# 2gunsu/monocon-pytorch

Measured on AMD Instinct MI355X. Metric: images/sec (384x1280) fwd+bwd, higher is better.
Workload: dtype f32 (f16x2); 1 GPU; train step B=32/GPU 3x384x1280 (configs[2] shape, fp32 values, mode f16x2); global_batch=32, parallelism=dp1, precision_mode=f16x2

## Files before the change

monocon-pytorch_amd/csrc/kernels_head_train.hip:

```cpp
#include <type_traits>

#include "kernels.h"
#include "train.h"

namespace mc {

__global__ void pack_conv_w_dgrad_kernel(const float *__restrict__ w, int Cout, int CinTotal, int k, int c_off, int Cs,
                                         int CsP, int CoutPad, int cls, float *__restrict__ dst) {
    const int kk = k * k;
    const size_t total = (size_t)Cout * Cs * kk;
    const int py = cls >> 1, px = cls & 1;
    for (size_t e = blockIdx.x * (size_t)blockDim.x + threadIdx.x; e < total; e += (size_t)gridDim.x * blockDim.x) {
        const int tap = e % kk;
        const int cl = (e / kk) % Cs;
        const int n = e / ((size_t)kk * Cs);
        const int r = tap / k, s = tap % k;
        int tapd;
        if (cls < 0) {
            tapd = (k - 1 - r) * k + (k - 1 - s);
        } else {
            if ((py == 0) != (r == 1) || (px == 0) != (s == 1)) continue;
            const int dr = py ? (2 - r) / 2 : 0, ds = px ? (2 - s) / 2 : 0;
            tapd = dr * (1 + px) + ds;
        }
        dst[(((size_t)tapd * (CoutPad >> 2) + (n >> 2)) * CsP + cl) * 4 + (n & 3)] =
            w[(((size_t)n * CinTotal + c_off + cl) * k + r) * k + s];
    }
}
hipError_t launch_pack_conv_w_dgrad(const float *w, int Cout, int CinTotal, int k, int c_off, int Cs, int CsP, int CoutPad,
                                    int cls, float *dst, hipStream_t st) {
    const size_t total = (size_t)Cout * Cs * k * k;
    size_t g = (total + 255) / 256;
    if (g > 4096) g = 4096;
    hipLaunchKernelGGL(pack_conv_w_dgrad_kernel, dim3((unsigned)g), dim3(256), 0, st, w, Cout, CinTotal, k, c_off, Cs, CsP,
                       CoutPad, cls, dst);
    return hipGetLastError();
}

struct HeadBwdArgs {
    const float *draw; int ld;
    const float *z, *x, *w1;
    const float *scale, *shift;
    float *d, *dw_partial, *red_partial;
    int HW, rows_per_block, blocks_per_img;
    const float *coef;
    float *csum;
    unsigned *amax;
};
constexpr int HB_PX = 64, HB_LD = 80;
constexpr int HB_WAVES = 4, HB_NT = HB_WAVES * 64, HB_MAXR = 24;

template <int RB, int NR, int MODE>
struct HeadPart {
    static constexpr int CP = NUM_HEADS * HEAD_CH;
    float w[NR], acc[NR];
    float s1, s2, zsc, zsh, cp, cq, cr;
    const float *xp, *zp;
    float *dp;
    bool rez;
    int h, sub, nsub;

    __device__ __forceinline__ void init(const HeadBwdArgs &a, int h_, int lane, size_t p0, int b, int sub_, int nsub_) {
        h = h_; sub = sub_; nsub = nsub_;
#pragma unroll
        for (int r = 0; r < NR; ++r) { w[r] = a.w1[(RB + r) * HEAD_CH + lane]; acc[r] = 0.f; }
        s1 = 0.f; s2 = 0.f;
        rez = a.z == nullptr;
        zsc = rez ? a.scale[(size_t)b * CP + h * HEAD_CH + lane] : 0.f;
        zsh = rez ? a.shift[(size_t)b * CP + h * HEAD_CH + lane] : 0.f;
        xp = a.x + p0 * CP + h * HEAD_CH + lane;
        zp = rez ? xp : a.z + p0 * CP + h * HEAD_CH + lane;
        dp = MODE == 1 ? nullptr : a.d + p0 * CP + h * HEAD_CH + lane;
        cp = cq = cr = 0.f;
        if (MODE == 2) {
            const float4 cf = reinterpret_cast<const float4 *>(a.coef)[(size_t)b * CP + h * HEAD_CH + lane];
            cp = cf.x; cq = cf.y; cr = cf.z;
        }
    }
    __device__ __forceinline__ void one(const float *gsh, int i, size_t gp, float zv, float xv) {
        const float *g = gsh + i * NR;
        float dh = 0.f;
#pragma unroll
        for (int r = 0; r < NR; ++r) {
            const float gv = g[r];
            if (MODE != 2) acc[r] = fmaf(gv, zv, acc[r]);
            dh = fmaf(gv, w[r], dh);
        }
        const float dv = zv > 0.f ? dh : 0.f;
        if (MODE == 2) {
            const float o = fmaf(cp, dv, fmaf(cq, xv, cr));
            s1 += o;
            s2 = fmaxf(s2, fabsf(o));
            dp[gp * CP] = o;
        } else {
            s1 += dv;
            s2 = fmaf(dv, xv, s2);
            if (MODE == 0) dp[gp * CP] = dv;
        }
    }
    __device__ __forceinline__ void block(const float *gsh, int px0, int n) {
        constexpr int U = NR > 8 ? 4 : 8;
        const int cnt = n > sub ? (n - sub + nsub - 1) / nsub : 0;
        int k = 0;
        for (; k + U <= cnt; k += U) {
            float zv[U], xv[U];
#pragma unroll
            for (int u = 0; u < U; ++u) {
                const size_t gp = (size_t)(px0 + sub + (k + u) * nsub);
                xv[u] = xp[gp * CP];
                if (!rez) zv[u] = zp[gp * CP];
            }
#pragma unroll
            for (int u = 0; u < U; ++u) {
                const int i = sub + (k + u) * nsub;
                one(gsh, i, (size_t)(px0 + i), rez ? fmaxf(fmaf(xv[u], zsc, zsh), 0.f) : zv[u], xv[u]);
                if (NR > 8) __builtin_amdgcn_sched_barrier(0);
            }
        }
        for (; k < cnt; ++k) {
            const int i = sub + k * nsub;
            const size_t gp = (size_t)(px0 + i);
            const float xv1 = xp[gp * CP];
            one(gsh, i, gp, rez ? fmaxf(fmaf(xv1, zsc, zsh), 0.f) : zp[gp * CP], xv1);
        }
    }
    __device__ __forceinline__ void spill(float *red, int lane) const {
        if (nsub == 1 || sub == 0) return;
        float *q = red + (size_t)(sub - 1) * (NR + 2) * 64 + lane;
        if (MODE != 2) {
#pragma unroll
            for (int r = 0; r < NR; ++r) q[r * 64] = acc[r];
        }
        q[NR * 64] = s1;
        q[(NR + 1) * 64] = s2;
    }
    __device__ __forceinline__ void finish(const HeadBwdArgs &a, const float *red, int blk, int lane) {
        if (MODE == 2 && a.amax) amax_update_wave(a.amax, s2);
        if (sub != 0) return;
        for (int k = 1; k < nsub; ++k) {
            const float *q = red + (size_t)(k - 1) * (NR + 2) * 64 + lane;
            if (MODE != 2) {
#pragma unroll
                for (int r = 0; r < NR; ++r) acc[r] += q[r * 64];
                s2 += q[(NR + 1) * 64];
            }
            s1 += q[NR * 64];
        }
        if (MODE == 2) {
            a.csum[((size_t)blk * CP + h * HEAD_CH + lane) * 2] = s1;
            return;
        }
#pragma unroll
        for (int r = 0; r < NR; ++r) a.dw_partial[((size_t)blk * NUM_OUT_ROWS + RB + r) * HEAD_CH + lane] = acc[r];
        float *rp = a.red_partial + ((size_t)blk * CP + h * HEAD_CH + lane) * 2;
        rp[0] = s1;
        rp[1] = s2;
    }
};

template <int RB, int NR, int MODE>
__device__ __forceinline__ void head_bwd_one(const HeadBwdArgs &a, float *gsh, float *red, int h, int wv, int lane, size_t p0, int np,
                                             int blk, int b) {
    HeadPart<RB, NR, MODE> P;
    P.init(a, h, lane, p0, b, wv, HB_WAVES);
    constexpr int NE = HB_PX * NR, NL = (NE + HB_NT - 1) / HB_NT;
    const int tid = threadIdx.x;
    const float *gsrc = a.draw + p0 * a.ld + RB;
    float pre[NL];
    auto fetch = [&](int px0) {
#pragma unroll
        for (int k = 0; k < NL; ++k) {
            const int e = tid + k * HB_NT, px = e / NR, r = e % NR;
            pre[k] = (e < NE && px0 + px < np) ? gsrc[(size_t)(px0 + px) * a.ld + r] : 0.f;
        }
    };
    fetch(0);
    for (int px0 = 0; px0 < np; px0 += HB_PX) {
        __syncthreads();
#pragma unroll
        for (int k = 0; k < NL; ++k) {
            const int e = tid + k * HB_NT;
            if (e < NE) gsh[e] = pre[k];
        }
        __syncthreads();
        if (px0 + HB_PX < np) fetch(px0 + HB_PX);
        P.block(gsh, px0, min(HB_PX, np - px0));
    }
    P.spill(red, lane);
    __syncthreads();
    P.finish(a, red, blk, lane);
}
template <int MODE, bool WIDE>
__global__ __launch_bounds__(HB_NT) void head_bwd_kernel(const HeadBwdArgs a) {
    __shared__ float gsh[HB_PX * (WIDE ? HB_MAXR : 3)];
    __shared__ float red[(HB_WAVES - 1) * ((WIDE ? HB_MAXR : 3) + 2) * 64];
    const int lane = threadIdx.x & 63;
    const int wv = __builtin_amdgcn_readfirstlane(threadIdx.x >> 6);
    const int blk = blockIdx.x;
    const int b = blk / a.blocks_per_img, rb = blk % a.blocks_per_img;
    const int r0 = rb * a.rows_per_block;
    const int np = min(a.HW, r0 + a.rows_per_block) - r0;
    const size_t p0 = (size_t)b * a.HW + r0;
    if (WIDE) {
        switch (blockIdx.y) {
            case 0: head_bwd_one<41, 24, MODE>(a, gsh, red, 8, wv, lane, p0, np, blk, b); break;
            case 1: head_bwd_one<7, 18, MODE>(a, gsh, red, 3, wv, lane, p0, np, blk, b); break;
            default: head_bwd_one<25, 9, MODE>(a, gsh, red, 4, wv, lane, p0, np, blk, b); break;
        }
    } else {
        switch (blockIdx.y) {
            case 0: head_bwd_one<0, 3, MODE>(a, gsh, red, 0, wv, lane, p0, np, blk, b); break;
            case 1: head_bwd_one<3, 2, MODE>(a, gsh, red, 1, wv, lane, p0, np, blk, b); break;
            case 2: head_bwd_one<5, 2, MODE>(a, gsh, red, 2, wv, lane, p0, np, blk, b); break;
            case 3: head_bwd_one<34, 2, MODE>(a, gsh, red, 5, wv, lane, p0, np, blk, b); break;
            case 4: head_bwd_one<36, 3, MODE>(a, gsh, red, 6, wv, lane, p0, np, blk, b); break;
            default: head_bwd_one<39, 2, MODE>(a, gsh, red, 7, wv, lane, p0, np, blk, b); break;
        }
    }
}
template <int MODE>
static void head_bwd_launch(const HeadBwdArgs &a, int blocks, hipStream_t st) {
    hipLaunchKernelGGL((head_bwd_kernel<MODE, true>), dim3(blocks, 3), dim3(HB_NT), 0, st, a);
    hipLaunchKernelGGL((head_bwd_kernel<MODE, false>), dim3(blocks, 6), dim3(HB_NT), 0, st, a);
}
static hipError_t head_bwd_args(HeadBwdArgs &a, const float *draw, int ld, const float *z, const float *x, const float *w1, int B,
                                int HW, int blocks, const float *scale, const float *shift) {
    const int *rbeg = head_row_begin();
    static const int RB[NUM_HEADS + 1] = {0, 3, 5, 7, 25, 34, 36, 39, 41, 65};
    for (int i = 0; i <= NUM_HEADS; ++i)
        if (rbeg[i] != RB[i]) return hipErrorInvalidValue;
    if (blocks % B || ld != HB_LD) return hipErrorInvalidValue;
    if (!z && (!scale || !shift)) return hipErrorInvalidValue;
    a = HeadBwdArgs{};
    a.draw = draw; a.ld = ld; a.z = z; a.x = x; a.w1 = w1;
    a.scale = scale; a.shift = shift;
    a.HW = HW; a.blocks_per_img = blocks / B; a.rows_per_block = (HW + a.blocks_per_img - 1) / a.blocks_per_img;
    return hipSuccess;
}
hipError_t launch_head_bwd(const float *draw, int ld, const float *z, const float *x, const float *w1, int B, int HW,
                           int blocks, float *d, float *dw_partial, float *red_partial, hipStream_t st, const float *scale,
                           const float *shift) {
    HeadBwdArgs a;
    hipError_t e = head_bwd_args(a, draw, ld, z, x, w1, B, HW, blocks, scale, shift);
    if (e != hipSuccess) return e;
    a.d = d; a.dw_partial = dw_partial; a.red_partial = red_partial;
    if (d) head_bwd_launch<0>(a, blocks, st);
    else head_bwd_launch<1>(a, blocks, st);
    return hipGetLastError();
}
hipError_t launch_head_dx(const float *draw, int ld, const float *x, const float *w1, const float *coef, int B, int HW, int blocks,
                          float *dx, float *csum, float *csum_out, unsigned *amax, hipStream_t st, const float *scale,
                          const float *shift) {
    if (!coef || !dx || !csum || !csum_out) return hipErrorInvalidValue;
    HeadBwdArgs a;
    hipError_t e = head_bwd_args(a, draw, ld, nullptr, x, w1, B, HW, blocks, scale, shift);
    if (e != hipSuccess) return e;
    a.d = dx; a.coef = coef; a.csum = csum; a.amax = amax;
    head_bwd_launch<2>(a, blocks, st);
    return launch_colsum_final(csum, blocks, NUM_HEADS * HEAD_CH, csum_out, st);
}


struct DpredPackArgs {
    const float *dpred[10];
    int ld, B, HW;
    float *out;
    int row_pred[NUM_OUT_ROWS], row_ch[NUM_OUT_ROWS], pred_c[10];
};
struct DpredUserArgs : DpredPackArgs {
    const float *grad[10];
    const float *pred[10];
    int row_epi[NUM_OUT_ROWS];
};
__device__ __forceinline__ float pred_act_grad(int epi, float y) {
    if (epi == 1) return (y > 1e-4f && y < 1.f - 1e-4f) ? y * (1.f - y) : 0.f;
    if (epi == 2) {
        const float sig = 1.f / (y + 1.f) - 1e-12f;
        return -sig * (1.f - sig) / ((sig + 1e-12f) * (sig + 1e-12f));
    }
    return 1.f;
}
template <bool USER>
__global__ __launch_bounds__(256) void dpred_pack_kernel(const std::conditional_t<USER, DpredUserArgs, DpredPackArgs> a) {
    __shared__ float t[64][NUM_OUT_ROWS + 2];
    __shared__ const float *rowp[NUM_OUT_ROWS];
    __shared__ const float *rowg[USER ? NUM_OUT_ROWS : 1], *rowy[USER ? NUM_OUT_ROWS : 1];
    __shared__ int rowe[USER ? NUM_OUT_ROWS : 1];
    const int tiles = (a.HW + 63) / 64;
    const int b = blockIdx.x / tiles, hw0 = (blockIdx.x % tiles) * 64;
    if (threadIdx.x < NUM_OUT_ROWS) {
        const int r = threadIdx.x, p = a.row_pred[r];
        rowp[r] = a.dpred[p] + ((size_t)b * a.pred_c[p] + a.row_ch[r]) * a.HW + hw0;
        if constexpr (USER) {
            const size_t o = ((size_t)b * a.pred_c[p] + a.row_ch[r]) * a.HW + hw0;
            rowg[r] = a.grad[p] ? a.grad[p] + o : nullptr;
            rowy[r] = a.pred[p] + o;
            rowe[r] = a.row_epi[r];
        }
    }
    __syncthreads();
    for (int e = threadIdx.x; e < 64 * NUM_OUT_ROWS; e += 256) {
        const int r = e / 64, px = e % 64;
        if constexpr (USER) {
            float v = 0.f;
            if (hw0 + px < a.HW) {
                v = rowp[r][px];
                if (rowg[r]) v += pred_act_grad(rowe[r], rowy[r][px]) * rowg[r][px];
            }
            t[px][r] = v;
        } else {
            t[px][r] = (hw0 + px < a.HW) ? rowp[r][px] : 0.f;
        }
    }
    __syncthreads();
    for (int e = threadIdx.x; e < 64 * a.ld; e += 256) {
        const int px = e / a.ld, r = e % a.ld;
        if (hw0 + px < a.HW) a.out[((size_t)b * a.HW + hw0 + px) * a.ld + r] = r < NUM_OUT_ROWS ? t[px][r] : 0.f;
    }
}
static void dpred_pack_args(DpredPackArgs &a, const float *const dpred[10], int ld, int B, int HW, float *out) {
    a.ld = ld; a.B = B; a.HW = HW; a.out = out;
    const HeadRow *rows = head_rows();
    for (int i = 0; i < 10; ++i) { a.dpred[i] = dpred[i]; a.pred_c[i] = PRED_CH[i]; }
    for (int r = 0; r < NUM_OUT_ROWS; ++r) { a.row_pred[r] = rows[r].pred; a.row_ch[r] = rows[r].ch; }
}
hipError_t launch_dpred_pack(const float *const dpred[10], int ld, int B, int HW, float *out, hipStream_t st) {
    DpredPackArgs a;
    dpred_pack_args(a, dpred, ld, B, HW, out);
    hipLaunchKernelGGL(dpred_pack_kernel<false>, dim3(B * ((HW + 63) / 64)), dim3(256), 0, st, a);
    return hipGetLastError();
}
hipError_t launch_dpred_pack_user(const float *const dpred[10], const float *const pred[10], const float *const grad[10], int ld,
                                  int B, int HW, float *out, hipStream_t st) {
    DpredUserArgs a;
    dpred_pack_args(a, dpred, ld, B, HW, out);
    const HeadRow *rows = head_rows();
    for (int i = 0; i < 10; ++i) {
        if (!pred[i]) return hipErrorInvalidValue;
        a.pred[i] = pred[i]; a.grad[i] = grad[i];
    }
    for (int r = 0; r < NUM_OUT_ROWS; ++r) a.row_epi[r] = rows[r].epi;
    hipLaunchKernelGGL(dpred_pack_kernel<true>, dim3(B * ((HW + 63) / 64)), dim3(256), 0, st, a);
    return hipGetLastError();
}

__device__ __forceinline__ float wave_sum(float v) {
#pragma unroll
    for (int o = 32; o > 0; o >>= 1) v += __shfl_xor(v, o);
    return v;
}

__device__ __forceinline__ void group_reduce2(double &s1, double &s2, double (*sh)[64][2], int grp, int c) {
    __syncthreads();
    sh[grp][c][0] = s1; sh[grp][c][1] = s2;
    __syncthreads();
    s1 = 0; s2 = 0;
#pragma unroll
    for (int g = 0; g < 16; ++g) { s1 += sh[g][c][0]; s2 += sh[g][c][1]; }
}

__global__ __launch_bounds__(1024) void inst_stats_kernel(const float *__restrict__ stats, int chunks, int stat_ld,
                                                          double *__restrict__ out) {
    const int b = blockIdx.x, c = threadIdx.x & 63, ch = blockIdx.y * 64 + c, part = threadIdx.x >> 6;
    const float2 *q = reinterpret_cast<const float2 *>(stats) + (size_t)b * chunks * stat_ld + ch;
    double s1 = 0.0, s2 = 0.0;
    int k = part;
    for (; k + 48 < chunks; k += 64) {
        const float2 v0 = q[(size_t)k * stat_ld], v1 = q[(size_t)(k + 16) * stat_ld], v2 = q[(size_t)(k + 32) * stat_ld],
                     v3 = q[(size_t)(k + 48) * stat_ld];
        s1 += (double)v0.x; s2 += (double)v0.y;
        s1 += (double)v1.x; s2 += (double)v1.y;
        s1 += (double)v2.x; s2 += (double)v2.y;
        s1 += (double)v3.x; s2 += (double)v3.y;
    }
    for (; k < chunks; k += 16) {
        const float2 v = q[(size_t)k * stat_ld];
        s1 += (double)v.x; s2 += (double)v.y;
    }
    __shared__ double red[2][16][64];
    red[0][part][c] = s1;
    red[1][part][c] = s2;
    __syncthreads();
    if (part < 2) {
        double t = 0.0;
#pragma unroll
        for (int g = 0; g < 16; ++g) t += red[part][g][c];
        out[((size_t)b * stat_ld + ch) * 2 + part] = t;
    }
}

__global__ __launch_bounds__(1024) void attn_train_fwd_kernel(const AttnTrainArgs a) {
    __shared__ double shred[16][64][2];
    const int h = blockIdx.x, c = threadIdx.x & 63, grp = threadIdx.x >> 6;
    const int CP = NUM_HEADS * HEAD_CH, ch = h * HEAD_CH + c;
    const double HW = (double)a.HW, n = HW * a.B;
    __shared__ float att[64][NUM_AFFINE];
    __shared__ float svl[64][HEAD_CH], awl[NUM_AFFINE][HEAD_CH];
    const float shift0 = a.rm[h][c];
    double S1 = 0, S2 = 0;
    double pre1[8], pre2[8];
    float aw[NUM_AFFINE], wk_[NUM_AFFINE], bk_[NUM_AFFINE];
#pragma unroll
    for (int k = 0; k < NUM_AFFINE; ++k) {
        aw[k] = a.att_w[h][k * HEAD_CH + c]; wk_[k] = a.weight_[h][k * HEAD_CH + c]; bk_[k] = a.bias_[h][k * HEAD_CH + c];
    }
    const int ck = c < NUM_AFFINE ? c : 0;
    const float att_g_c = a.att_g[h][ck], att_b_c = a.att_b[h][ck], att_rm_c = a.att_rm[h][ck], att_rv_c = a.att_rv[h][ck];
    const float rv_c = a.rv[h][c];
    for (int b = 0; b < a.B; ++b) {
        double s1 = 0, s2 = 0;
        if (a.stats64) {
            if ((b & 7) == 0) {
#pragma unroll
                for (int u = 0; u < 8; ++u) {
                    const int bb = b + u < a.B ? b + u : a.B - 1;
                    const double2 v = *reinterpret_cast<const double2 *>(a.stats64 + ((size_t)bb * a.stat_ld + ch) * 2);
                    pre1[u] = v.x; pre2[u] = v.y;
                }
// ... 501 lines not shown
```

monocon-pytorch_amd/csrc/mc_train_plan.hip:

```cpp
#include <atomic>
#include <deque>
#include <functional>

#include "mc_internal.h"

using namespace mc;

namespace {

using Fn = std::function<int(mc_handle *, hipStream_t)>;

struct PlanSwitches {
    long long lazy_z;
    long long lazy_min;
    long long lazy_feat;
    long long zbits;
    long long grad_pool;
    long long grad_pool_cool;
    long long head_dx_fuse;
    long long dgrad_s2_thin;
    long long stem_fuse;
    long long bm_epilogue;
    long long wres_bwd;
    long long dual_stream;
    int side_sync_lo = 0, side_sync_hi = 0;
    bool plan_debug = false;
};
const struct { const char *name; long long PlanSwitches::*field; long long def; } SWITCH_TABLE[] = {
    {"MONOCON_HIP_LAZY_Z", &PlanSwitches::lazy_z, 3},
    {"MONOCON_HIP_LAZY_MIN", &PlanSwitches::lazy_min, 900000},
    {"MONOCON_HIP_LAZY_FEAT", &PlanSwitches::lazy_feat, 0},
    {"MONOCON_HIP_ZBITS", &PlanSwitches::zbits, 1},
    {"MONOCON_HIP_GRAD_POOL", &PlanSwitches::grad_pool, 1},
    {"MONOCON_HIP_GRAD_POOL_COOL", &PlanSwitches::grad_pool_cool, 2},
    {"MONOCON_HIP_HEAD_DX_FUSE", &PlanSwitches::head_dx_fuse, 1},
    {"MONOCON_HIP_DGRAD_S2_THIN", &PlanSwitches::dgrad_s2_thin, 1},
    {"MONOCON_HIP_STEM_FUSE", &PlanSwitches::stem_fuse, 1},
    {"MONOCON_HIP_BM_EPILOGUE", &PlanSwitches::bm_epilogue, 1},
    {"MONOCON_HIP_WRES_BWD", &PlanSwitches::wres_bwd, 0},
    {"MONOCON_HIP_DUAL_STREAM", &PlanSwitches::dual_stream, 1},
};
PlanSwitches read_switches() {
    PlanSwitches sw{};
    std::string changed;
    for (const auto &d : SWITCH_TABLE) {
        const char *e = std::getenv(d.name);
        sw.*d.field = e ? std::atoll(e) : d.def;
        if (sw.*d.field != d.def) changed += std::string(" ") + d.name + "=" + std::to_string(sw.*d.field);
    }
    if (const char *e = std::getenv("MONOCON_HIP_SIDE_SYNC")) {
        if (std::sscanf(e, "%d:%d", &sw.side_sync_lo, &sw.side_sync_hi) != 2) sw.side_sync_lo = sw.side_sync_hi = 0;
        if (sw.side_sync_lo < sw.side_sync_hi) changed += std::string(" MONOCON_HIP_SIDE_SYNC=") + e;
    }
    sw.plan_debug = std::getenv("MONOCON_HIP_PLAN_DEBUG") != nullptr;
    if (sw.plan_debug && !changed.empty()) fprintf(stderr, "[plan] switches off their defaults:%s\n", changed.c_str());
    return sw;
}

struct PoolBwdArgs {
    const float *x, *dout, *la, *lb;
    float *dx, *stats;
    int B, H, W, C, acc;
};

struct LastWriter {
    enum Kind { NONE, DGRAD_CONV, POOL_BWD, DECONV_BWD } kind = NONE;
    union {
        ConvArgs *conv;
        PoolBwdArgs *pool;
        float **deconv_stats;
    };
    LastWriter() : conv(nullptr) {}
    LastWriter(ConvArgs *c) : kind(c ? DGRAD_CONV : NONE), conv(c) {}
    LastWriter(PoolBwdArgs *p) : kind(p ? POOL_BWD : NONE), pool(p) {}
    LastWriter(float **s) : kind(s ? DECONV_BWD : NONE), deconv_stats(s) {}
};

struct TNode {
    Tensor t;
    float *g = nullptr;
    bool ginit = false, needs_grad = true;
    LastWriter last;
    const float *la = nullptr, *lb = nullptr;
    bool lrelu = true;
};

struct PackJob {
    const float *w;
    int Cout, CinTotal, k, c_off, Cs, CsP, CoutPad;
    int cls;
    float *dst;
    void *dst16;
    unsigned *amax;
};

enum RecKind { REC_STEM, REC_CONV, REC_POOL, REC_DECONV, REC_HEAD };
struct Rec {
    RecKind kind;
    ConvLayer *L = nullptr;
    DeconvLayer *D = nullptr;
    std::vector<int> srcs;
    int res = -1, z = -1, in = -1;
    bool relu = true, dead = false;
    Tensor y;
    float *mean = nullptr, *rstd = nullptr;
    float *ca = nullptr, *cb = nullptr;
    unsigned *zbits = nullptr;
    std::string bn;
};

enum BwdStream { ON_MAIN, ON_SIDE };
struct BwdStep {
    Fn fn;
    BwdStream stream = ON_MAIN;
    int wait = -1;
    int bucket = -1;
    bool feat_dgrad = false;
    bool img_dgrad = false;
// ... 546 lines not shown
            at.att_w[hd] = P(an + ".attn_weights.attention.0.weight", AC);
            at.att_g[hd] = P(an + ".attn_weights.attention.1.weight", A);
            at.att_b[hd] = P(an + ".attn_weights.attention.1.bias", A);
            at.att_rm[hd] = P(an + ".attn_weights.attention.1.running_mean", A);
            at.att_rv[hd] = P(an + ".attn_weights.attention.1.running_var", A);
            at.att_nbt[hd] = NBT(an + ".attn_weights.attention.1.num_batches_tracked");
            at.weight_[hd] = P(an + ".weight_", AC); at.bias_[hd] = P(an + ".bias_", AC);
            gp.d_weight_[hd] = G(an + ".weight_", AC); gp.d_bias_[hd] = G(an + ".bias_", AC);
            gp.d_att_w[hd] = G(an + ".attn_weights.attention.0.weight", AC);
            gp.d_att_g[hd] = G(an + ".attn_weights.attention.1.weight", A);
            gp.d_att_b[hd] = G(an + ".attn_weights.attention.1.bias", A);
        }
        ConvArgs c3{};
        c3.nsrc = 1;
        fill_src(c3.src[0], feat);
        const TNode &fn = ts->nodes[feat];
        c3.B = B; c3.Hin = fh; c3.Win = fw; c3.Hout = fh; c3.Wout = fw; c3.Cin = 64; c3.Cout = CP; c3.CoutP = h->head3.coutp;
        c3.wpk = h->head3.wpk; c3.bias = h->head_bias; c3.out = xh.p; c3.out_ld = CP; c3.cfg = h->head3.cfg;
        c3.wpk16 = h->head3.wpk16; c3.prec = h->prec;
        if (h->prec == 3) { c3.amax_in[0] = fn.t.amax; c3.amax_w = h->head3.w_amax; }
        if (c3.src[0].la && (!fn.lrelu || !conv_lazy_capable(c3, 3, 1))) {
            materialise(feat);
            fill_src(c3.src[0], feat);
        }
        at.chunks = conv_chunks_per_image(c3.cfg, fh, fw);
        at.stat_ld = h->head3.coutp;
        float *stats = alloc((size_t)B * at.chunks * at.stat_ld * 2);
        c3.stats = stats; c3.stat_shift = h->head_rm;
        at.stats = stats; at.B = B; at.HW = HW;
        at.stats64 = reinterpret_cast<double *>(alloc((size_t)B * at.stat_ld * 4));
        at.sv_inst = alloc((size_t)B * CP * 3); at.mu_r = alloc((size_t)CP * 2); at.bn10 = alloc(NUM_HEADS * NUM_AFFINE * 2);
        at.that = alloc((size_t)B * NUM_HEADS * NUM_AFFINE); at.yatt = alloc((size_t)B * NUM_HEADS * NUM_AFFINE);
        at.gamma_p = alloc((size_t)B * CP); at.scale = alloc((size_t)B * CP); at.shift = alloc((size_t)B * CP);
        w3dense = alloc((size_t)CP * 64 * 9);
        HeadApplyArgs ha{};
        ha.hidden = xh.p; ha.scale = at.scale; ha.shift = at.shift; ha.w = h->head_w1t; ha.b = h->head_b1;
        ha.B = B; ha.HW = HW; ha.z_out = nullptr;
        for (int i = 0; i < 10; ++i) ha.pred_c[i] = PRED_CH[i];
        ts->fwd.push_back([=](mc_handle *hh, hipStream_t st) { HIPCHK(hh, launch_conv(c3, 3, 1, st)); return 0; });
        ts->fwd.push_back([=, ts = ts, at = at](mc_handle *hh, hipStream_t st) {
            HIPCHK(hh, launch_attn_train_fwd(at, st));
            HeadApplyArgs a2 = ha;
            for (int i = 0; i < 10; ++i) a2.pred[i] = ts->preds[i];
            HIPCHK(hh, launch_head_apply(a2, st));
            return 0;
        });
    }

    void targets_and_losses() {
        mc_targets &T = ts->targets;
        const size_t R = (size_t)B * ts->max_objs;
        auto up = [](size_t n) { return (n + 63) / 64 * 64; };
        const size_t tn[15] = {(size_t)B * 3 * HW, (size_t)B * 9 * HW, R * 2, R * 2, R * 3, R, R, R, R * 18, R * 18,
                               R * 2, R * 18, R / 4 + 1, R * 18, R * 18};
        size_t ttot = 0;
        for (size_t n : tn) ttot += up(n);
        float *ta = alloc(ttot);
        float *tp[15];
        { size_t o = 0; for (int i = 0; i < 15; ++i) { tp[i] = ta ? ta + o : nullptr; o += up(tn[i]); } }
        T.center_heatmap_target = tp[0]; T.kpt_heatmap_target = tp[1];
        T.wh_target = tp[2]; T.offset_target = tp[3]; T.dim_target = tp[4];
        T.alpha_cls_target = tp[5]; T.alpha_offset_target = tp[6]; T.depth_target = tp[7];
        T.center2kpt_offset_target = tp[8]; T.kpt_heatmap_offset_target = tp[9];
        T.indices = reinterpret_cast<int64_t *>(tp[10]); T.indices_kpt = reinterpret_cast<int64_t *>(tp[11]);
        T.mask_target = reinterpret_cast<uint8_t *>(tp[12]);
        T.mask_center2kpt_offset = tp[13]; T.mask_kpt_heatmap_offset = tp[14];
        h->tgt_arena = ta; h->tgt_arena_bytes = ttot * sizeof(float);
        ts->dpred[0] = alloc((size_t)B * PRED_CH[0] * HW);
        ts->dpred[1] = alloc((size_t)B * PRED_CH[1] * HW);
        size_t dtot = 0;
        for (int i = 2; i < 10; ++i) dtot += up((size_t)B * PRED_CH[i] * HW);
        float *da = alloc(dtot);
        { size_t o = 0; for (int i = 2; i < 10; ++i) { ts->dpred[i] = da ? da + o : nullptr; o += up((size_t)B * PRED_CH[i] * HW); } }
        h->dp_arena = da; h->dp_arena_bytes = dtot * sizeof(float);
        ts->fwd.push_back([ts = ts, B = B, fh = fh, fw = fw](mc_handle *hh, hipStream_t st) {
            if (mc_make_targets(hh, &ts->labels, B, ts->max_objs, ts->pad_h, ts->pad_w, fh, fw, &ts->targets, st)) return -1;
            if (mc_losses(hh, ts->preds, &ts->targets, B, ts->max_objs, fh, fw, ts->losses, st)) return -1;
            return 0;
        });
    }

    void heads_backward(int feat) {
        float *draw = alloc(raw_numel);
        float *cs1 = alloc(colsum_partial_floats((size_t)B * HW, LD));
        float *db1 = alloc(NUM_OUT_ROWS), *dw1 = alloc((size_t)NUM_OUT_ROWS * HEAD_CH);
        push_bwd([=, ts = ts, B = B, fh = fh, fw = fw, HW = HW](mc_handle *hh, hipStream_t st) {
            if (mc_losses_backward(hh, ts->preds, &ts->targets, B, ts->max_objs, fh, fw, ts->grad_losses, ts->dpred, st)) return -1;
            bool user = false;
            for (const float *g : ts->grad_preds) user = user || g != nullptr;
            if (user)
                HIPCHK(hh, launch_dpred_pack_user(ts->dpred, ts->preds, ts->grad_preds, LD, B, HW, draw, st));
            else
                HIPCHK(hh, launch_dpred_pack(ts->dpred, LD, B, HW, draw, st));
            HIPCHK(hh, launch_colsum(draw, (size_t)B * HW, NUM_OUT_ROWS, LD, cs1, db1, st));
            return 0;
        });
        const int nbr = chan_reduce_blocks(B, HW), rb_per_img = nbr / B;
        const bool dx_fuse = sw.head_dx_fuse != 0;
        float *dh = alloc(xh.numel());
        float *dw1p = alloc((size_t)nbr * NUM_OUT_ROWS * HEAD_CH);
        float *partial = alloc((size_t)nbr * CP * 2), *coef = alloc((size_t)B * CP * 4);
        float *dx = dh;
        const int *rb = head_row_begin();
        CopyBatch segcb;
        auto seg = [&](const std::string &layer, int r0, int nr) {
            if (!segcb.add(dw1 + (size_t)r0 * HEAD_CH, G(layer + ".weight", nr * HEAD_CH), (size_t)nr * HEAD_CH) ||
                !segcb.add(db1 + r0, G(layer + ".bias", nr), nr))
                ts->ok = false;
        };
        for (int hd = 0; hd < 8; ++hd) seg(std::string("head.") + HEAD_NAMES[hd] + ".3", rb[hd], rb[hd + 1] - rb[hd]);
        seg("head.dir_cls.0", rb[8], 12);
        seg("head.dir_reg.0", rb[8] + 12, 12);
        const float *xp = xh.p, *w1 = h->head_w1, *zsc = at.scale, *zsh = at.shift;
        push_bwd([=, B = B, HW = HW](mc_handle *hh, hipStream_t st) {
            HIPCHK(hh, launch_head_bwd(draw, LD, nullptr, xp, w1, B, HW, nbr, dx_fuse ? nullptr : dh, dw1p, partial, st, zsc, zsh));
            HIPCHK(hh, launch_splitk_reduce(dw1p, nbr, 1, NUM_OUT_ROWS, HEAD_CH, dw1, st));
            HIPCHK(hh, launch_copy_batch(segcb, st));
            return 0;
        });
        float *db3 = alloc(CP), *dw3 = alloc((size_t)CP * 64 * 9);
        float *cs3 = alloc((size_t)std::max(affine_bwd_blocks(B, (size_t)HW, CP), nbr) * CP * 2);
        Tensor dxT = xh; dxT.p = dx; dxT.amax = slot();
        unsigned *dxmax = dxT.amax;
        push_bwd([=, at = at, gp = gp, B = B, HW = HW](mc_handle *hh, hipStream_t st) {
            HIPCHK(hh, launch_attn_train_bwd(at, partial, rb_per_img, gp, coef, st));
            if (dx_fuse)
                HIPCHK(hh, launch_head_dx(draw, LD, xp, w1, coef, B, HW, nbr, dx, cs3, db3, dxmax, st, zsc, zsh));
            else
                HIPCHK(hh, launch_affine_bwd(dh, nullptr, xp, coef, B, (size_t)HW, CP, 1, 0, dx, nullptr, 0, st, nullptr, nullptr, cs3, db3,
                                             dxmax));
            return 0;
        });
        emit_wgrad({feat}, dxT, CP, CP, 3, 1, dw3);
        CopyBatch g3cb;
        for (int hd = 0; hd < NUM_HEADS; ++hd) {
            const std::string layer = std::string("head.") + HEAD_NAMES[hd] + ".0";
            if (!g3cb.add(dw3 + (size_t)hd * 64 * 64 * 9, G(layer + ".weight", 9 * HEAD_CH * HEAD_CH), (size_t)64 * 64 * 9) ||
                !g3cb.add(db3 + hd * 64, G(layer + ".bias", HEAD_CH), 64))
                ts->ok = false;
        }
        push_bwd([=](mc_handle *hh, hipStream_t st) { HIPCHK(hh, launch_copy_batch(g3cb, st)); return 0; }, ON_SIDE);
        CopyBatch w3cb;
        for (int hd = 0; hd < NUM_HEADS; ++hd)
            if (!w3cb.add(P(std::string("head.") + HEAD_NAMES[hd] + ".0.weight", 9 * HEAD_CH * HEAD_CH), w3dense + (size_t)hd * 64 * 64 * 9,
                          (size_t)64 * 64 * 9))
                ts->ok = false;
        ts->pack_fns.push_back([=](mc_handle *hh, hipStream_t st) { HIPCHK(hh, launch_copy_batch(w3cb, st)); return 0; });
        if (h->prec == 3) h->w_amax_of[w3dense] = h->head3.w_amax;
        emit_dgrad(w3dense, dxT, CP, 64, 3, 1, 0, feat, CP);
        if (ts->head_only) ts->bwd.back().feat_dgrad = true;
    }

    void pool_backward(const Rec &r) {
        TNode &in = ts->nodes[r.in];
        const TNode &o = ts->nodes[r.z];
        if (!o.ginit || !in.needs_grad) return;
        float *gi = g_acquire(r.in);
        PoolBwdArgs pa{in.t.p, o.g, in.la, in.lb, gi, nullptr, in.t.B, in.t.H, in.t.W, in.t.C, in.ginit ? 1 : 0};
        ts->pool_bwds.push_back(pa);
        PoolBwdArgs *pp = &ts->pool_bwds.back();
        push_bwd([=](mc_handle *hh, hipStream_t st) {
            HIPCHK(hh, launch_maxpool2_bwd(pp->x, pp->dout, pp->B, pp->H, pp->W, pp->C, pp->dx, pp->acc, st, pp->la, pp->lb, pp->stats));
            return 0;
        });
        wrote(r.in, pp);
        g_release(r.z, -1);
    }

    void deconv_backward(const Rec &r) {
        TNode &in = ts->nodes[r.in];
        const TNode &o = ts->nodes[r.z];
        if (!o.ginit) return;
        if (in.ginit) { ts->ok = false; h->err = "train plan: deconv input has more than one consumer"; }
        const float *xp = in.t.p, *go = o.g, *wp = r.D->wpk, *xla = in.la, *xlb = in.lb;
        float *gi = g_acquire(r.in), *dw = G(r.D->name + ".weight", (int64_t)r.D->C * 16);
        const int Bq = in.t.B, Hq = in.t.H, Wq = in.t.W, Cq = in.t.C;
        float *part = alloc(deconv4_bwd_w_partial_floats(Bq, Hq, Cq));
        ts->deconv_stats.push_back(nullptr);
        float **dstats = &ts->deconv_stats.back();
        push_bwd([=](mc_handle *hh, hipStream_t st) {
            HIPCHK(hh, launch_deconv4_bwd_w(xp, go, Bq, Hq, Wq, Cq, part, dw, st, xla, xlb, wp, gi, *dstats));
            return 0;
        });
        wrote(r.in, (xla && xlb) ? dstats : nullptr);
        g_release(r.z, -1);
    }

    void conv_backward(const Rec &r) {
        if (r.dead || !ts->nodes[r.z].ginit) return;
        const Tensor dy = bn_backward(r, r.bn).dy;
        const int64_t wn = (int64_t)r.L->cout * r.L->cin * r.L->ks * r.L->ks;
        const int wgrad = emit_wgrad(r.srcs, dy, r.L->cout, r.L->cout, r.L->ks, r.L->stride, G(r.L->conv + ".weight", wn));
        const float *wm = P(r.L->conv + ".weight", wn);
        int c_off = 0;
        for (int s : r.srcs) {
            emit_dgrad(wm, dy, r.L->cout, r.L->cin, r.L->ks, r.L->stride, c_off, s, r.L->cout);
            c_off += ts->nodes[s].t.C;
        }
        g_release(r.z, wgrad);
    }

    void stem_backward(const Rec &r) {
        if (!ts->nodes[r.z].ginit) return;
        const bool want_fused = sw.stem_fuse && h->prec == 3 && ts->img_amax && r.y.amax && W % 4 == 0 && W >= 16;
        const BnBwd bb = bn_backward(r, r.bn, want_fused);
        const bool fused = bb.affine_skipped;
        float *part = alloc((size_t)stem_wgrad_blocks(B, H, W) * 147 * 16), *dw = G("backbone.base_layer.0.weight", 16 * 147);
        const float *dyp = bb.dy.p, *yfp = fused ? r.y.p : nullptr, *cfp = fused ? bb.coef : nullptr;
        const unsigned *imax = ts->img_amax, *dymax = bb.dy.amax, *yfmax = fused ? r.y.amax : nullptr;
        const int wgrad = push_bwd([=, ts = ts, B = B, H = H, W = W](mc_handle *hh, hipStream_t st) {
// ... 372 lines not shown
```

monocon-pytorch_amd/csrc/train.h:

```cpp
#pragma once
#include <hip/hip_runtime.h>
#include <stdint.h>
#include <vector>

#include "conv_mfma.h"

namespace mc {

struct TargetArgs {
    const float *gt_bboxes, *gt_labels, *gt_bboxes_3d, *depths, *gt_kpts_2d, *gt_kpts_valid, *mask;
    int B, max_objs, num_kpt, num_classes, fh, fw;
    float h_ratio, w_ratio;
    float *center_heatmap, *kpt_heatmap;
    float *wh, *offset, *dim, *alpha_cls, *alpha_offset, *depth, *c2k, *kho;
    long long *indices, *indices_kpt;
    uint8_t *mask_target;
    float *mask_c2k, *mask_kho;
};
hipError_t launch_make_targets(const TargetArgs &a, hipStream_t st);

hipError_t launch_focal(const float *p, const float *t, size_t n, float *partial, float *loss_out, float *aux,
                        hipStream_t st);
hipError_t launch_focal_grad(const float *p, const float *t, size_t n, const float *aux, const float *gscale, int gidx,
                             float *dlogit, hipStream_t st, int wrt_pred = 0);
// ... 26 lines not shown
    int CoutP;
    int n_off, c_off;
    int CsP, cls, nsplit;
    int block_begin, nblocks;
    unsigned *amax;
};
struct PackBatch {
    std::vector<PackJobDesc> jobs;
    PackJobDesc *dev = nullptr;
    int total_blocks = 0;
    bool uploaded = false;
    void clear();
    void add(PackJobDesc j);
    hipError_t launch(hipStream_t st, bool with_amax = false);
    PackBatch() = default;
    PackBatch(const PackBatch &) = delete;
    PackBatch &operator=(const PackBatch &) = delete;
    ~PackBatch();
};
struct FoldJobDesc {
    const float *g, *b, *rm, *rv;
    float eps;
    int C;
    float *scale, *shift;
};
struct FoldBatch {
    std::vector<FoldJobDesc> jobs;
    FoldJobDesc *dev = nullptr;
    bool uploaded = false;
    int maxC = 0;
    void clear();
    void add(const FoldJobDesc &j);
    hipError_t launch(hipStream_t st);
    FoldBatch() = default;
    FoldBatch(const FoldBatch &) = delete;
    FoldBatch &operator=(const FoldBatch &) = delete;
    ~FoldBatch();
};

struct OptTensor { float *p, *g, *m, *v; };
struct OptChunk { int tensor, begin, count; };
struct AdamHyper { float decay, beta1, one_minus_beta1, beta2, one_minus_beta2, sqrt_bc2, eps, step_size; };
hipError_t launch_clip_adamw(const OptTensor *tab, const OptChunk *chunks, int nchunks, float *partial, float *normcoef,
                             float max_norm, const AdamHyper &hp, hipStream_t st);
int opt_partial_floats();

int chan_reduce_blocks(int B, int rows_per_img);
hipError_t launch_chan_reduce(const float *y, const float *dz, const float *z, const float *shift, int B, int rows_per_img,
                              int C, int mode, int relu, float *partial, int Cstride, hipStream_t st, const float *fa = nullptr,
                              const float *fb = nullptr);
hipError_t launch_bn_finalize(const float *partial, int nb, int Cstride, double n, int C, const float *shift,
                              const float *gamma, const float *beta, float eps, float momentum, float *rm, float *rv,
                              long long *nbt, float *a, float *b, float *mean, float *rstd, hipStream_t st,
                              double *fold = nullptr, const unsigned *ymax = nullptr, unsigned *zmax = nullptr, int zrelu = 1);
size_t partial_fold_doubles(int nb, int C);
hipError_t launch_affine_act(const float *y, const float *a, const float *b, const float *res, int B, size_t rows_per_img,
                             int C, int per_sample, int relu, float *z, hipStream_t st, unsigned *amax = nullptr,
                             const float *res_a = nullptr, const float *res_b = nullptr, int res_relu = 0,
                             unsigned *zbits = nullptr);
hipError_t launch_bn_bwd_finalize(const float *partial, int nb, int Cstride, double n, int C, const float *gamma,
                                  const float *mean, const float *rstd, float *dgamma, float *dbeta, float *coef,
                                  hipStream_t st, double *fold = nullptr);
hipError_t launch_affine_bwd(const float *dz, const float *z, const float *y, const float *coef, int B, size_t rows_per_img,
                             int C, int per_sample, int relu, float *dy, float *gres, int gres_mode, hipStream_t st,
                             const float *fa = nullptr, const float *fb = nullptr, float *csum = nullptr, float *csum_out = nullptr,
                             unsigned *amax = nullptr);
int affine_bwd_blocks(int B, size_t rows_per_img, int C);
hipError_t launch_add(float *a, const float *b, size_t n, hipStream_t st);
size_t colsum_partial_floats(size_t rows, int ld);
hipError_t launch_colsum(const float *x, size_t rows, int C, int ld, float *partial, float *out, hipStream_t st);
hipError_t launch_colsum_final(const float *partial, int nb, int C, float *out, hipStream_t st);
hipError_t launch_maxpool2_bwd(const float *x, const float *dout, int B, int H, int W, int C, float *dx, int accumulate,
                               hipStream_t st, const float *la = nullptr, const float *lb = nullptr,
                               float *stats_partial = nullptr);
int maxpool2_bwd_blocks(int B, int H, int W, int C);
size_t deconv4_bwd_w_partial_floats(int B, int H, int C);
hipError_t launch_deconv4_bwd_w(const float *in, const float *dout, int B, int H, int W, int C, float *partial, float *dw,
                                hipStream_t st, const float *la, const float *lb,
                                const float *wpk, float *din,
                                float *stats = nullptr);

hipError_t launch_pack_conv_w_dgrad(const float *w, int Cout, int CinTotal, int k, int c_off, int Cs, int CsP, int CoutPad,
                                    int cls, float *dst, hipStream_t st);
hipError_t launch_dpred_pack(const float *const dpred[10], int ld, int B, int HW, float *out, hipStream_t st);
hipError_t launch_dpred_pack_user(const float *const dpred[10], const float *const pred[10], const float *const grad[10], int ld,
                                  int B, int HW, float *out, hipStream_t st);
struct AttnTrainArgs {
    const float *stats;
    int chunks, stat_ld, B, HW;
    double *stats64;
    float *rm[9], *rv[9];
    long long *nbt[9];
    const float *att_w[9], *att_g[9], *att_b[9];
    float *att_rm[9], *att_rv[9];
    long long *att_nbt[9];
    const float *weight_[9], *bias_[9];
    float *sv_inst;
    float *mu_r;
    float *bn10;
    float *that, *yatt;
    float *gamma_p;
    float *scale, *shift;
};
struct AttnGradPtrs { float *d_weight_[9], *d_bias_[9], *d_att_w[9], *d_att_g[9], *d_att_b[9]; };
hipError_t launch_attn_train_fwd(const AttnTrainArgs &a, hipStream_t st);
hipError_t launch_attn_train_bwd(const AttnTrainArgs &a, const float *partial, int rb_per_img, const AttnGradPtrs &gp,
                                 float *coef, hipStream_t st);
hipError_t launch_head_bwd(const float *draw, int ld, const float *z, const float *x, const float *w1, int B, int HW,
                           int blocks, float *d, float *dw_partial, float *red_partial, hipStream_t st,
                           const float *scale = nullptr, const float *shift = nullptr);
hipError_t launch_head_dx(const float *draw, int ld, const float *x, const float *w1, const float *coef, int B, int HW, int blocks,
                          float *dx, float *csum, float *csum_out, unsigned *amax, hipStream_t st, const float *scale,
                          const float *shift);
hipError_t launch_splitk_reduce(const float *partial, int ksplit, int T, int Cout, int Cin, float *dw, hipStream_t st);
int stem_wgrad_blocks(int B, int H, int W);
hipError_t launch_stem_wgrad(const float *img, const float *dy, int B, int H, int W, float *partial, float *dw,
                             hipStream_t st, const unsigned *img_amax = nullptr, const unsigned *dy_amax = nullptr,
                             const float *y = nullptr, const float *coef = nullptr, const unsigned *y_amax = nullptr);
hipError_t launch_stem_dgrad(const float *dy, const float *w_oihw, int B, int H, int W, float *dx, hipStream_t st,
                             const float *y = nullptr, const float *coef = nullptr);

struct WgradArgs {
    ConvSrc src[4];
    int nsrc;
    int B, Hin, Win, Hout, Wout, Cin, Cout;
    const float *dy;
    int dy_ld;
    float *partial;
    int ksplit, n_tiles, c_tiles, ppr, ppi, groups_per_img;
    int small;
    int prec;
    int pb;
    int pipe;
    const unsigned *amax_x[4], *amax_dy;
};
void wgrad_plan(WgradArgs &a, int ks, int stride);
size_t wgrad_partial_floats(const WgradArgs &a, int ks);
hipError_t launch_wgrad(const WgradArgs &a, int ks, int stride, float *dw_oihw, hipStream_t st);
bool wgrad_lazy_capable(const WgradArgs &a, int ks, int stride);
bool wgrad_bf16_ok(const WgradArgs &a, int ks, int stride);
hipError_t launch_wgrad_bf16(const WgradArgs &a, int ks, int stride, int WN, int WC, hipStream_t st);
int wgrad_bf16_patches(int prec);
int wgrad_pipe_tile(const WgradArgs &a, int ks, int stride);
void wgrad_pipe_plan(WgradArgs &a, int tile);
hipError_t launch_wgrad_pipe(const WgradArgs &a, int ks, hipStream_t st);
bool wgrad_thin_ok(const WgradArgs &a, int ks, int stride);
hipError_t launch_wgrad_thin(const WgradArgs &a, hipStream_t st);

}
```

Measured before the change: 662.7 images/sec.

## Skip zero-gradient head tiles in head backward via per-tile nonzero masks

The dpred pack kernel now records, per 64-pixel tile and image, a bitmask of which heads have any nonzero incoming gradient. The head backward and head dx kernels read this mask and, for tiles whose head gradient is all zero, skip the shared-memory staging, barriers and per-row accumulation. In those tiles they only write zeros, or the affine term in dx mode. This targets sparse head gradients such as heatmap or regression losses that are nonzero only near objects. It adds an atomicOr and a wave vote in the pack kernel, plus extra control flow.

```diff
diff --git a/monocon-pytorch_amd/csrc/kernels_head_train.hip b/monocon-pytorch_amd/csrc/kernels_head_train.hip
--- a/monocon-pytorch_amd/csrc/kernels_head_train.hip
+++ b/monocon-pytorch_amd/csrc/kernels_head_train.hip
@@ -39,6 +39,7 @@
 
 struct HeadBwdArgs {
     const float *draw; int ld;
+    const unsigned *nz; int nz_tiles;
     const float *z, *x, *w1;
     const float *scale, *shift;
     float *d, *dw_partial, *red_partial;
@@ -48,6 +49,16 @@
     unsigned *amax;
 };
 constexpr int HB_PX = 64, HB_LD = 80;
+static bool head_rows_as_coded() {
+    const int *rbeg = head_row_begin();
+    static const int RB[NUM_HEADS + 1] = {0, 3, 5, 7, 25, 34, 36, 39, 41, 65};
+    for (int i = 0; i <= NUM_HEADS; ++i)
+        if (rbeg[i] != RB[i]) return false;
+    return true;
+}
+__device__ __forceinline__ int head_of_row(int r) {
+    return (r >= 3) + (r >= 5) + (r >= 7) + (r >= 25) + (r >= 34) + (r >= 36) + (r >= 39) + (r >= 41);
+}
 constexpr int HB_WAVES = 4, HB_NT = HB_WAVES * 64, HB_MAXR = 24;
 
 template <int RB, int NR, int MODE>
@@ -124,6 +135,35 @@
             one(gsh, i, gp, rez ? fmaxf(fmaf(xv1, zsc, zsh), 0.f) : zp[gp * CP], xv1);
         }
     }
+    __device__ __forceinline__ void zero_block(int px0, int n) {
+        if (MODE == 1) return;
+        const int cnt = n > sub ? (n - sub + nsub - 1) / nsub : 0;
+        if (MODE == 0) {
+            for (int k = 0; k < cnt; ++k) dp[(size_t)(px0 + sub + k * nsub) * CP] = 0.f;
+            return;
+        }
+        constexpr int U = 8;
+        int k = 0;
+        for (; k + U <= cnt; k += U) {
+            float xv[U];
+#pragma unroll
+            for (int u = 0; u < U; ++u) xv[u] = xp[(size_t)(px0 + sub + (k + u) * nsub) * CP];
+#pragma unroll
+            for (int u = 0; u < U; ++u) {
+                const float o = fmaf(cq, xv[u], cr);
+                s1 += o;
+                s2 = fmaxf(s2, fabsf(o));
+                dp[(size_t)(px0 + sub + (k + u) * nsub) * CP] = o;
+            }
+        }
+        for (; k < cnt; ++k) {
+            const size_t gp = (size_t)(px0 + sub + k * nsub);
+            const float o = fmaf(cq, xp[gp * CP], cr);
+            s1 += o;
+            s2 = fmaxf(s2, fabsf(o));
+            dp[gp * CP] = o;
+        }
+    }
     __device__ __forceinline__ void spill(float *red, int lane) const {
         if (nsub == 1 || sub == 0) return;
         float *q = red + (size_t)(sub - 1) * (NR + 2) * 64 + lane;
@@ -160,9 +200,16 @@
 
 template <int RB, int NR, int MODE>
 __device__ __forceinline__ void head_bwd_one(const HeadBwdArgs &a, float *gsh, float *red, int h, int wv, int lane, size_t p0, int np,
-                                             int blk, int b) {
+                                             int blk, int b, int r0) {
     HeadPart<RB, NR, MODE> P;
     P.init(a, h, lane, p0, b, wv, HB_WAVES);
+    const unsigned *nzb = a.nz ? a.nz + (size_t)b * a.nz_tiles : nullptr;
+    auto live = [&](int px0) -> bool {
+        if (!nzb) return true;
+        const int first = r0 + px0, last = r0 + min(px0 + HB_PX, np) - 1;
+        const unsigned m = nzb[first >> 6] | nzb[last >> 6];
+        return (__builtin_amdgcn_readfirstlane(m) >> h) & 1u;
+    };
     constexpr int NE = HB_PX * NR, NL = (NE + HB_NT - 1) / HB_NT;
     const int tid = threadIdx.x;
     const float *gsrc = a.draw + p0 * a.ld + RB;
@@ -174,17 +221,25 @@
             pre[k] = (e < NE && px0 + px < np) ? gsrc[(size_t)(px0 + px) * a.ld + r] : 0.f;
         }
     };
-    fetch(0);
+    bool cur = np > 0 && live(0);
+    if (cur) fetch(0);
     for (int px0 = 0; px0 < np; px0 += HB_PX) {
-        __syncthreads();
-#pragma unroll
-        for (int k = 0; k < NL; ++k) {
-            const int e = tid + k * HB_NT;
-            if (e < NE) gsh[e] = pre[k];
-        }
-        __syncthreads();
-        if (px0 + HB_PX < np) fetch(px0 + HB_PX);
-        P.block(gsh, px0, min(HB_PX, np - px0));
+        const bool nxt = px0 + HB_PX < np && live(px0 + HB_PX);
+        if (cur) {
+            __syncthreads();
+#pragma unroll
+            for (int k = 0; k < NL; ++k) {
+                const int e = tid + k * HB_NT;
+                if (e < NE) gsh[e] = pre[k];
+            }
+            __syncthreads();
+            if (nxt) fetch(px0 + HB_PX);
+            P.block(gsh, px0, min(HB_PX, np - px0));
+        } else {
+            if (nxt) fetch(px0 + HB_PX);
+            P.zero_block(px0, min(HB_PX, np - px0));
+        }
+        cur = nxt;
     }
     P.spill(red, lane);
     __syncthreads();
@@ -203,18 +258,18 @@
     const size_t p0 = (size_t)b * a.HW + r0;
     if (WIDE) {
         switch (blockIdx.y) {
-            case 0: head_bwd_one<41, 24, MODE>(a, gsh, red, 8, wv, lane, p0, np, blk, b); break;
-            case 1: head_bwd_one<7, 18, MODE>(a, gsh, red, 3, wv, lane, p0, np, blk, b); break;
-            default: head_bwd_one<25, 9, MODE>(a, gsh, red, 4, wv, lane, p0, np, blk, b); break;
+            case 0: head_bwd_one<41, 24, MODE>(a, gsh, red, 8, wv, lane, p0, np, blk, b, r0); break;
+            case 1: head_bwd_one<7, 18, MODE>(a, gsh, red, 3, wv, lane, p0, np, blk, b, r0); break;
+            default: head_bwd_one<25, 9, MODE>(a, gsh, red, 4, wv, lane, p0, np, blk, b, r0); break;
         }
     } else {
         switch (blockIdx.y) {
-            case 0: head_bwd_one<0, 3, MODE>(a, gsh, red, 0, wv, lane, p0, np, blk, b); break;
-            case 1: head_bwd_one<3, 2, MODE>(a, gsh, red, 1, wv, lane, p0, np, blk, b); break;
-            case 2: head_bwd_one<5, 2, MODE>(a, gsh, red, 2, wv, lane, p0, np, blk, b); break;
-            case 3: head_bwd_one<34, 2, MODE>(a, gsh, red, 5, wv, lane, p0, np, blk, b); break;
-            case 4: head_bwd_one<36, 3, MODE>(a, gsh, red, 6, wv, lane, p0, np, blk, b); break;
-            default: head_bwd_one<39, 2, MODE>(a, gsh, red, 7, wv, lane, p0, np, blk, b); break;
+            case 0: head_bwd_one<0, 3, MODE>(a, gsh, red, 0, wv, lane, p0, np, blk, b, r0); break;
+            case 1: head_bwd_one<3, 2, MODE>(a, gsh, red, 1, wv, lane, p0, np, blk, b, r0); break;
+            case 2: head_bwd_one<5, 2, MODE>(a, gsh, red, 2, wv, lane, p0, np, blk, b, r0); break;
+            case 3: head_bwd_one<34, 2, MODE>(a, gsh, red, 5, wv, lane, p0, np, blk, b, r0); break;
+            case 4: head_bwd_one<36, 3, MODE>(a, gsh, red, 6, wv, lane, p0, np, blk, b, r0); break;
+            default: head_bwd_one<39, 2, MODE>(a, gsh, red, 7, wv, lane, p0, np, blk, b, r0); break;
         }
     }
 }
@@ -224,24 +279,22 @@
     hipLaunchKernelGGL((head_bwd_kernel<MODE, false>), dim3(blocks, 6), dim3(HB_NT), 0, st, a);
 }
 static hipError_t head_bwd_args(HeadBwdArgs &a, const float *draw, int ld, const float *z, const float *x, const float *w1, int B,
-                                int HW, int blocks, const float *scale, const float *shift) {
-    const int *rbeg = head_row_begin();
-    static const int RB[NUM_HEADS + 1] = {0, 3, 5, 7, 25, 34, 36, 39, 41, 65};
-    for (int i = 0; i <= NUM_HEADS; ++i)
-        if (rbeg[i] != RB[i]) return hipErrorInvalidValue;
+                                int HW, int blocks, const float *scale, const float *shift, const unsigned *nz) {
+    if (!head_rows_as_coded()) return hipErrorInvalidValue;
     if (blocks % B || ld != HB_LD) return hipErrorInvalidValue;
     if (!z && (!scale || !shift)) return hipErrorInvalidValue;
     a = HeadBwdArgs{};
     a.draw = draw; a.ld = ld; a.z = z; a.x = x; a.w1 = w1;
     a.scale = scale; a.shift = shift;
+    a.nz = nz; a.nz_tiles = (HW + 63) / 64;
     a.HW = HW; a.blocks_per_img = blocks / B; a.rows_per_block = (HW + a.blocks_per_img - 1) / a.blocks_per_img;
     return hipSuccess;
 }
 hipError_t launch_head_bwd(const float *draw, int ld, const float *z, const float *x, const float *w1, int B, int HW,
                            int blocks, float *d, float *dw_partial, float *red_partial, hipStream_t st, const float *scale,
-                           const float *shift) {
+                           const float *shift, const unsigned *nz) {
     HeadBwdArgs a;
-    hipError_t e = head_bwd_args(a, draw, ld, z, x, w1, B, HW, blocks, scale, shift);
+    hipError_t e = head_bwd_args(a, draw, ld, z, x, w1, B, HW, blocks, scale, shift, nz);
     if (e != hipSuccess) return e;
     a.d = d; a.dw_partial = dw_partial; a.red_partial = red_partial;
     if (d) head_bwd_launch<0>(a, blocks, st);
@@ -250,10 +303,10 @@
 }
 hipError_t launch_head_dx(const float *draw, int ld, const float *x, const float *w1, const float *coef, int B, int HW, int blocks,
                           float *dx, float *csum, float *csum_out, unsigned *amax, hipStream_t st, const float *scale,
-                          const float *shift) {
+                          const float *shift, const unsigned *nz) {
     if (!coef || !dx || !csum || !csum_out) return hipErrorInvalidValue;
     HeadBwdArgs a;
-    hipError_t e = head_bwd_args(a, draw, ld, nullptr, x, w1, B, HW, blocks, scale, shift);
+    hipError_t e = head_bwd_args(a, draw, ld, nullptr, x, w1, B, HW, blocks, scale, shift, nz);
     if (e != hipSuccess) return e;
     a.d = dx; a.coef = coef; a.csum = csum; a.amax = amax;
     head_bwd_launch<2>(a, blocks, st);
@@ -265,6 +318,7 @@
     const float *dpred[10];
     int ld, B, HW;
     float *out;
+    unsigned *nz;
     int row_pred[NUM_OUT_ROWS], row_ch[NUM_OUT_ROWS], pred_c[10];
 };
 struct DpredUserArgs : DpredPackArgs {
@@ -286,6 +340,8 @@
     __shared__ const float *rowp[NUM_OUT_ROWS];
     __shared__ const float *rowg[USER ? NUM_OUT_ROWS : 1], *rowy[USER ? NUM_OUT_ROWS : 1];
     __shared__ int rowe[USER ? NUM_OUT_ROWS : 1];
+    __shared__ unsigned nzw;
+    if (threadIdx.x == 0) nzw = 0u;
     const int tiles = (a.HW + 63) / 64;
     const int b = blockIdx.x / tiles, hw0 = (blockIdx.x % tiles) * 64;
     if (threadIdx.x < NUM_OUT_ROWS) {
@@ -299,41 +355,47 @@
         }
     }
     __syncthreads();
+    unsigned nzm = 0u;
     for (int e = threadIdx.x; e < 64 * NUM_OUT_ROWS; e += 256) {
         const int r = e / 64, px = e % 64;
+        float v = 0.f;
         if constexpr (USER) {
-            float v = 0.f;
             if (hw0 + px < a.HW) {
                 v = rowp[r][px];
                 if (rowg[r]) v += pred_act_grad(rowe[r], rowy[r][px]) * rowg[r][px];
             }
-            t[px][r] = v;
         } else {
-            t[px][r] = (hw0 + px < a.HW) ? rowp[r][px] : 0.f;
-        }
-    }
-    __syncthreads();
+            if (hw0 + px < a.HW) v = rowp[r][px];
+        }
+        t[px][r] = v;
+        if (__any(v != 0.f)) nzm |= 1u << head_of_row(r);
+    }
+    if (a.nz && (threadIdx.x & 63) == 0 && nzm) atomicOr(&nzw, nzm);
+    __syncthreads();
+    if (a.nz && threadIdx.x == 0) a.nz[blockIdx.x] = nzw;
     for (int e = threadIdx.x; e < 64 * a.ld; e += 256) {
         const int px = e / a.ld, r = e % a.ld;
         if (hw0 + px < a.HW) a.out[((size_t)b * a.HW + hw0 + px) * a.ld + r] = r < NUM_OUT_ROWS ? t[px][r] : 0.f;
     }
 }
-static void dpred_pack_args(DpredPackArgs &a, const float *const dpred[10], int ld, int B, int HW, float *out) {
-    a.ld = ld; a.B = B; a.HW = HW; a.out = out;
+static void dpred_pack_args(DpredPackArgs &a, const float *const dpred[10], int ld, int B, int HW, float *out, unsigned *nz) {
+    a.ld = ld; a.B = B; a.HW = HW; a.out = out; a.nz = nz;
     const HeadRow *rows = head_rows();
     for (int i = 0; i < 10; ++i) { a.dpred[i] = dpred[i]; a.pred_c[i] = PRED_CH[i]; }
     for (int r = 0; r < NUM_OUT_ROWS; ++r) { a.row_pred[r] = rows[r].pred; a.row_ch[r] = rows[r].ch; }
 }
-hipError_t launch_dpred_pack(const float *const dpred[10], int ld, int B, int HW, float *out, hipStream_t st) {
+hipError_t launch_dpred_pack(const float *const dpred[10], int ld, int B, int HW, float *out, hipStream_t st, unsigned *nz) {
+    if (nz && !head_rows_as_coded()) return hipErrorInvalidValue;
     DpredPackArgs a;
-    dpred_pack_args(a, dpred, ld, B, HW, out);
+    dpred_pack_args(a, dpred, ld, B, HW, out, nz);
     hipLaunchKernelGGL(dpred_pack_kernel<false>, dim3(B * ((HW + 63) / 64)), dim3(256), 0, st, a);
     return hipGetLastError();
 }
 hipError_t launch_dpred_pack_user(const float *const dpred[10], const float *const pred[10], const float *const grad[10], int ld,
-                                  int B, int HW, float *out, hipStream_t st) {
+                                  int B, int HW, float *out, hipStream_t st, unsigned *nz) {
+    if (nz && !head_rows_as_coded()) return hipErrorInvalidValue;
     DpredUserArgs a;
-    dpred_pack_args(a, dpred, ld, B, HW, out);
+    dpred_pack_args(a, dpred, ld, B, HW, out, nz);
     const HeadRow *rows = head_rows();
     for (int i = 0; i < 10; ++i) {
         if (!pred[i]) return hipErrorInvalidValue;
diff --git a/monocon-pytorch_amd/csrc/mc_train_plan.hip b/monocon-pytorch_amd/csrc/mc_train_plan.hip
--- a/monocon-pytorch_amd/csrc/mc_train_plan.hip
+++ b/monocon-pytorch_amd/csrc/mc_train_plan.hip
@@ -18,6 +18,7 @@
     long long grad_pool;
     long long grad_pool_cool;
     long long head_dx_fuse;
+    long long head_zskip;
     long long dgrad_s2_thin;
     long long stem_fuse;
     long long bm_epilogue;
@@ -34,6 +35,7 @@
     {"MONOCON_HIP_GRAD_POOL", &PlanSwitches::grad_pool, 1},
     {"MONOCON_HIP_GRAD_POOL_COOL", &PlanSwitches::grad_pool_cool, 2},
     {"MONOCON_HIP_HEAD_DX_FUSE", &PlanSwitches::head_dx_fuse, 1},
+    {"MONOCON_HIP_HEAD_ZSKIP", &PlanSwitches::head_zskip, 1},
     {"MONOCON_HIP_DGRAD_S2_THIN", &PlanSwitches::dgrad_s2_thin, 1},
     {"MONOCON_HIP_STEM_FUSE", &PlanSwitches::stem_fuse, 1},
     {"MONOCON_HIP_BM_EPILOGUE", &PlanSwitches::bm_epilogue, 1},
@@ -746,6 +748,12 @@
 
     void heads_backward(int feat) {
         float *draw = alloc(raw_numel);
+        const size_t nz_words = (size_t)B * ((HW + 63) / 64);
+        unsigned *nz = sw.head_zskip ? reinterpret_cast<unsigned *>(alloc(nz_words)) : nullptr;
+        const unsigned *nz_bwd = nz, *nz_dx = sw.head_zskip == 1 ? nz : nullptr;
+        if (sw.plan_debug)
+            fprintf(stderr, "[plan] heads backward: zero-tile skip %s (%zu tile words)\n",
+                    !sw.head_zskip ? "off" : sw.head_zskip == 1 ? "on" : "on in the statistics pass only", sw.head_zskip ? nz_words : (size_t)0);
         float *cs1 = alloc(colsum_partial_floats((size_t)B * HW, LD));
         float *db1 = alloc(NUM_OUT_ROWS), *dw1 = alloc((size_t)NUM_OUT_ROWS * HEAD_CH);
         push_bwd([=, ts = ts, B = B, fh = fh, fw = fw, HW = HW](mc_handle *hh, hipStream_t st) {
@@ -753,9 +761,9 @@
             bool user = false;
             for (const float *g : ts->grad_preds) user = user || g != nullptr;
             if (user)
-                HIPCHK(hh, launch_dpred_pack_user(ts->dpred, ts->preds, ts->grad_preds, LD, B, HW, draw, st));
+                HIPCHK(hh, launch_dpred_pack_user(ts->dpred, ts->preds, ts->grad_preds, LD, B, HW, draw, st, nz));
             else
-                HIPCHK(hh, launch_dpred_pack(ts->dpred, LD, B, HW, draw, st));
+                HIPCHK(hh, launch_dpred_pack(ts->dpred, LD, B, HW, draw, st, nz));
             HIPCHK(hh, launch_colsum(draw, (size_t)B * HW, NUM_OUT_ROWS, LD, cs1, db1, st));
             return 0;
         });
@@ -777,7 +785,7 @@
         seg("head.dir_reg.0", rb[8] + 12, 12);
         const float *xp = xh.p, *w1 = h->head_w1, *zsc = at.scale, *zsh = at.shift;
         push_bwd([=, B = B, HW = HW](mc_handle *hh, hipStream_t st) {
-            HIPCHK(hh, launch_head_bwd(draw, LD, nullptr, xp, w1, B, HW, nbr, dx_fuse ? nullptr : dh, dw1p, partial, st, zsc, zsh));
+            HIPCHK(hh, launch_head_bwd(draw, LD, nullptr, xp, w1, B, HW, nbr, dx_fuse ? nullptr : dh, dw1p, partial, st, zsc, zsh, nz_bwd));
             HIPCHK(hh, launch_splitk_reduce(dw1p, nbr, 1, NUM_OUT_ROWS, HEAD_CH, dw1, st));
             HIPCHK(hh, launch_copy_batch(segcb, st));
             return 0;
@@ -789,7 +797,7 @@
         push_bwd([=, at = at, gp = gp, B = B, HW = HW](mc_handle *hh, hipStream_t st) {
             HIPCHK(hh, launch_attn_train_bwd(at, partial, rb_per_img, gp, coef, st));
             if (dx_fuse)
-                HIPCHK(hh, launch_head_dx(draw, LD, xp, w1, coef, B, HW, nbr, dx, cs3, db3, dxmax, st, zsc, zsh));
+                HIPCHK(hh, launch_head_dx(draw, LD, xp, w1, coef, B, HW, nbr, dx, cs3, db3, dxmax, st, zsc, zsh, nz_dx));
             else
                 HIPCHK(hh, launch_affine_bwd(dh, nullptr, xp, coef, B, (size_t)HW, CP, 1, 0, dx, nullptr, 0, st, nullptr, nullptr, cs3, db3,
                                              dxmax));
diff --git a/monocon-pytorch_amd/csrc/train.h b/monocon-pytorch_amd/csrc/train.h
--- a/monocon-pytorch_amd/csrc/train.h
+++ b/monocon-pytorch_amd/csrc/train.h
@@ -132,9 +132,10 @@
 
 hipError_t launch_pack_conv_w_dgrad(const float *w, int Cout, int CinTotal, int k, int c_off, int Cs, int CsP, int CoutPad,
                                     int cls, float *dst, hipStream_t st);
-hipError_t launch_dpred_pack(const float *const dpred[10], int ld, int B, int HW, float *out, hipStream_t st);
+hipError_t launch_dpred_pack(const float *const dpred[10], int ld, int B, int HW, float *out, hipStream_t st,
+                             unsigned *nz = nullptr);
 hipError_t launch_dpred_pack_user(const float *const dpred[10], const float *const pred[10], const float *const grad[10], int ld,
-                                  int B, int HW, float *out, hipStream_t st);
+                                  int B, int HW, float *out, hipStream_t st, unsigned *nz = nullptr);
 struct AttnTrainArgs {
     const float *stats;
     int chunks, stat_ld, B, HW;
@@ -158,10 +159,10 @@
                                  float *coef, hipStream_t st);
 hipError_t launch_head_bwd(const float *draw, int ld, const float *z, const float *x, const float *w1, int B, int HW,
                            int blocks, float *d, float *dw_partial, float *red_partial, hipStream_t st,
-                           const float *scale = nullptr, const float *shift = nullptr);
+                           const float *scale = nullptr, const float *shift = nullptr, const unsigned *nz = nullptr);
 hipError_t launch_head_dx(const float *draw, int ld, const float *x, const float *w1, const float *coef, int B, int HW, int blocks,
                           float *dx, float *csum, float *csum_out, unsigned *amax, hipStream_t st, const float *scale,
-                          const float *shift);
+                          const float *shift, const unsigned *nz = nullptr);
 hipError_t launch_splitk_reduce(const float *partial, int ksplit, int T, int Cout, int Cin, float *dw, hipStream_t st);
 int stem_wgrad_blocks(int B, int H, int W);
 hipError_t launch_stem_wgrad(const float *img, const float *dy, int B, int H, int W, float *partial, float *dw,
```

Measured after the change: 672.0 images/sec, median of 6. +1.4%, better.
